# choi403/ALG

Measured on AMD Instinct MI355X. Metric: frames/sec (whole node) CogVideoX-5B-I2V 49f x 50-step ALG, higher is better.
Workload: dtype bf16; 1 GPU; BASELINE config 2: CogVideoX-5B-I2V bf16, 49 frames @ 480x720, 50 steps, ALG interval down_up (resize_factor 0.25, interval [0, 0.04]), guidance 6.0; one video per GPU; layers=42, dit_sample_forwards=12, parallelism=dp1

## Files before the change

alg_amd/_lib.py:

```python
from __future__ import annotations

import ctypes
from collections import OrderedDict
import os
from ctypes import POINTER, Structure, byref, c_char_p, c_float, c_int, c_int32, c_int64, c_void_p

import torch

_HERE = os.path.dirname(os.path.abspath(__file__))
LIB_PATH = os.environ.get("ALG_HIP_LIB") or os.path.join(_HERE, "libalg_hip.so")

ALG_F32, ALG_BF16 = 0, 1
ACT_NONE, ACT_GELU_TANH, ACT_SILU = 0, 1, 2
GEMM_BIAS_PER_ROW, GEMM_PERMUTE_COLS, GEMM_GATE_F32, GEMM_GATE_SEG_STRIDE = 1, 4, 8, 16
GEMM_B_PACKED11 = 32

EXPORTS = (
    "alg_version", "alg_last_error", "alg_reload_env", "alg_down_up", "alg_gaussian_blur", "alg_cfg_ddim_step", "alg_gemm_bf16", "alg_gemm_bf16_pair", "alg_gemm_bf16_pair_qk", "alg_pack_b_p11", "alg_pack_b_p11_bytes",
    "alg_flash_attn_d64", "alg_layernorm_modulate", "alg_layernorm_modulate_fp8", "alg_qk_norm_rope", "alg_patchify", "alg_unpatchify",
    "alg_timestep_embedding", "alg_cfg_combine", "alg_lincomb", "alg_unipc_update", "alg_concat_cast", "alg_flash_attn_d128", "alg_layernorm_mod_f32", "alg_layernorm_mod_f32_fp8", "alg_rmsnorm_rope",
    "alg_wan_modulation", "alg_patchify3d", "alg_unpatchify3d", "alg_timestep_embedding_f32", "alg_linear_f32",
    "alg_gelu_erf", "alg_layernorm_modulate_seg", "alg_headnorm_rope", "alg_masked_mean", "alg_silu", "alg_gemm_fp8", "alg_quantize_fp8_rows",
    "alg_conv_cl_bf16", "alg_vae_groupnorm_workspace", "alg_vae_groupnorm_stats", "alg_vae_spatial_norm", "alg_vae_upsample",
    "alg_vae_pack_latent", "alg_vae_unpack_video", "alg_vae_group_norm", "alg_vae_pad", "alg_vae_repitch",
    "alg_vae_unpack_planes", "alg_rms_norm_rows", "alg_softmax_hilo", "alg_flash_attn_d128_ex", "alg_flash_attn_d128_dual", "alg_rope_half", "alg_patchify_t", "alg_unpatchify_t", "alg_qk_norm_rope_scaled", "alg_flash_attn_d64_ex", "alg_embed_rows", "alg_t5_layernorm", "alg_attn_bias", "alg_mul_bf16", "alg_quick_gelu",
    "alg_lowpass_tables_bytes", "alg_lowpass_tables_build", "alg_down_up_workspace_bytes", "alg_gaussian_blur_workspace_bytes",
    "alg_flash_attn_d64_workspace_bytes", "alg_calib_mfma_bf16", "alg_wall_clock_khz", "alg_attn_clock_tap", "alg_attn_path_tap",
    "alg_flash_attn_d128_fp8", "alg_quantize_fp8_khead", "alg_quantize_fp8_vt", "alg_rmsnorm_rope_fp8", "alg_headnorm_rope_fp8",
    "alg_layernorm_modulate_seg_fp8", "alg_quantize_fp8_rows_batched", "alg_step_cache_probe", "alg_step_cache_workspace_bytes",
    "alg_flash_attn_d128_ranges", "alg_flash_attn_d64_ranges", "alg_flash_attn_d128_ranges_heads", "alg_attn_lse_recall", "alg_flash_attn_d64_ranges_heads",
    "alg_flash_attn_d128_ranges_order", "alg_flash_attn_d64_ranges_order",
    "alg_flash_attn_d128_ranges_prefix", "alg_attn_prefix_mass",
    "alg_gemm_fp4", "alg_quantize_mxfp4_rows", "alg_gemm_fp4_q4out", "alg_layernorm_modulate_mxfp4",
    "alg_attn_rows_position_major", "alg_attn_vt_position_major",
)
_RET_I64 = ("alg_vae_groupnorm_workspace", "alg_lowpass_tables_bytes", "alg_down_up_workspace_bytes",
            "alg_gaussian_blur_workspace_bytes", "alg_flash_attn_d64_workspace_bytes", "alg_pack_b_p11_bytes",
            "alg_step_cache_workspace_bytes")


class AlgHipError(RuntimeError):
    pass


class GemmArgs(Structure):
    _fields_ = [
        ("A", c_void_p), ("B", c_void_p), ("C", c_void_p), ("bias", c_void_p), ("R", c_void_p), ("gate", c_void_p),
        ("lda", c_int64), ("ldb", c_int64), ("ldc", c_int64), ("ldr", c_int64),
        ("strideA", c_int64), ("strideB", c_int64), ("strideC", c_int64), ("strideR", c_int64),
# ... 120 lines not shown
    lib.alg_t5_layernorm.argtypes = [c_void_p, c_void_p, c_void_p, c_int64, c_int, c_float, c_void_p]
    lib.alg_attn_bias.argtypes = [c_void_p] * 7 + [c_int, c_int, c_int, c_int, c_int64, c_int64, c_float, c_int, c_void_p]
    lib.alg_quick_gelu.argtypes = [c_void_p, c_int64, c_void_p]
    lib.alg_mul_bf16.argtypes = [c_void_p, c_void_p, c_void_p, c_int64, c_void_p]
    lib.alg_vae_upsample.argtypes = [c_void_p, c_void_p] + [c_int] * 6 + [c_void_p]
    lib.alg_vae_pack_latent.argtypes = [c_void_p, c_int64, c_int64, c_void_p, c_int, c_int, c_int, c_int, c_float, c_void_p]
    lib.alg_vae_unpack_video.argtypes = [c_void_p, c_void_p, c_int, c_int, c_int, c_int, c_void_p]
    lib.alg_quantize_fp8_rows.argtypes = [c_void_p, c_int64, c_void_p, c_void_p, c_int64, c_int, c_void_p]
    lib.alg_timestep_embedding_f32.argtypes = [c_void_p, c_void_p, c_int, c_int, c_void_p]
    lib.alg_linear_f32.argtypes = [c_void_p] * 6 + [c_int] * 4 + [c_void_p]
    lib.alg_gelu_erf.argtypes = [c_void_p, c_int64, c_void_p]
    lib.alg_unipc_update.argtypes = [c_void_p] * 5 + [c_int64] + [c_float] * 6 + [c_void_p]
    lib.alg_gemm_bf16.argtypes = [POINTER(GemmArgs), c_void_p]
    lib.alg_gemm_bf16_pair.argtypes = [POINTER(GemmArgs), POINTER(GemmArgs), c_void_p]
    lib.alg_gemm_bf16_pair_qk.argtypes = [POINTER(GemmArgs), POINTER(GemmArgs), POINTER(QkNormRopeArgs), c_void_p]
    lib.alg_flash_attn_d64.argtypes = [c_void_p, c_void_p, c_void_p, c_void_p, c_int, c_int, c_int, c_int64, c_int64,
                                       c_int64, c_int64, c_int64, c_int64, c_float, c_void_p]
    lib.alg_layernorm_modulate.argtypes = [c_void_p, c_void_p, c_void_p, c_void_p, c_void_p, c_void_p, c_int64, c_int,
                                           c_int, c_int, c_int64, c_int64, c_int, c_float, c_void_p]
    lib.alg_layernorm_modulate_fp8.argtypes = [c_void_p] * 7 + [c_int64, c_int, c_int, c_int, c_int64, c_int, c_float, c_void_p]
    lib.alg_layernorm_modulate_seg_fp8.argtypes = [c_void_p] * 7 + [c_int64, c_int64, c_int, c_int, c_int, c_int64, c_int, c_float,
                                                   c_void_p]
    lib.alg_quantize_fp8_rows_batched.argtypes = [c_void_p, c_int64, c_int64, c_void_p, c_void_p, c_int, c_int, c_int, c_void_p]
    lib.alg_qk_norm_rope.argtypes = [c_void_p, c_void_p, c_void_p, c_void_p, c_void_p, c_void_p, c_void_p, c_int,
                                     c_int, c_int, c_int, c_float, c_void_p]
    lib.alg_qk_norm_rope_scaled.argtypes = [c_void_p] * 7 + [c_int, c_int, c_int, c_int, c_float, c_float, c_void_p]
    lib.alg_flash_attn_d64_ex.argtypes = [c_void_p, c_void_p, c_void_p, c_void_p, c_int, c_int, c_int, c_int64, c_int64,
                                          c_int64, c_int64, c_int64, c_int64, c_float, c_int, c_void_p, c_int64, c_void_p]
    lib.alg_flash_attn_d64_ranges.argtypes = [c_void_p] * 4 + [c_int] * 3 + [c_int64] * 6 + [c_void_p, c_int, c_void_p]
    lib.alg_flash_attn_d64_ranges_heads.argtypes = ([c_void_p] * 4 + [c_int] * 3 + [c_int64] * 6 +
# ... 821 lines not shown
    lib = load_library()
    args, fp8 = gemm_args(*a, **kw)
    if fp8:
        _check(lib.alg_gemm_fp8(ctypes.byref(args), _stream()), "alg_gemm_fp8")
    else:
        _check(lib.alg_gemm_bf16(ctypes.byref(args), _stream()), "alg_gemm_bf16")


def gemm_pair(first, second):
    lib = load_library()
    a, fa = gemm_args(*first[0], **first[1])
    b, fb = gemm_args(*second[0], **second[1])
    if fa or fb:
        raise AlgHipError("gemm_pair takes bf16 problems")
    _check(lib.alg_gemm_bf16_pair(ctypes.byref(a), ctypes.byref(b), _stream()), "alg_gemm_bf16_pair")


def gemm_pair_qk(first, second, wq, bq, wk, bk, cos, sin, heads, text_len, eps, q_scale=1.0):
    lib = load_library()
    a, fa = gemm_args(*first[0], **first[1])
    b, fb = gemm_args(*second[0], **second[1])
    if fa or fb:
        raise AlgHipError("gemm_pair_qk takes bf16 problems")
    ptrs = [t.data_ptr() if t is not None else None for t in (wq, bq, wk, bk, cos, sin)]
    e = QkNormRopeArgs(*ptrs, heads, text_len, float(eps), float(q_scale))
    _check(lib.alg_gemm_bf16_pair_qk(ctypes.byref(a), ctypes.byref(b), ctypes.byref(e), _stream()), "alg_gemm_bf16_pair_qk")


def quantize_fp8_rows(x, q, scale, rows, K, x_rstride=None, x_off=0, q_off=0, scale_off=0):
    x_rstride = K if x_rstride is None else x_rstride
# ... 234 lines not shown
```

alg_amd/csrc/gemm.hip:

```cpp
#include <stdlib.h>

#include "common.h"

namespace alg {
constexpr int BM = 256, BN = 256;
typedef int launch_one_fn(const alg_gemm_args* a, int m_tiles, int n_tiles, int64_t nwg, hipStream_t s);
typedef int launch_pair_fn(const alg_gemm_args* a, int m_tiles_a, int n_tiles_a, const alg_gemm_args* b, int m_tiles_b, int n_tiles_b,
                           const alg_qk_norm_rope_args* e, hipStream_t s);
launch_one_fn launch_gemm_p6, launch_gemm_p6_conv, launch_gemm_p6_fp8, launch_gemm_p9, launch_gemm_p9_fp8, launch_gemm_p10, launch_gemm_p11;
launch_pair_fn launch_gemm_p9_pair, launch_gemm_p10_pair;
static int gemm_pipe() { return opt(OPT_GEMM_PIPE); }

static bool asm_loop_takes(int K, int64_t ld, int64_t esz) {
  return K * esz >= 256 && 256 * ld * esz + K * esz < (1ll << 32);
}

enum GemmRoute { ROUTE_P6, ROUTE_P6_CONV, ROUTE_P6_FP8, ROUTE_P9, ROUTE_P9_FP8, ROUTE_P10, ROUTE_P11 };
struct GemmPlan {
  GemmRoute route;
  int m_tiles, n_tiles;
  int64_t nwg;
  bool slabs;
  bool pairable;
};
}
// ... 160 lines not shown
}
static int pair_launch(const alg_gemm_args* a, const alg_gemm_args* b, const PairPlan& pp, const alg_qk_norm_rope_args* e, void* stream) {
  return (pp.a.route == ROUTE_P10 ? launch_gemm_p10_pair : launch_gemm_p9_pair)(a, pp.a.m_tiles, pp.a.n_tiles, b, pp.b.m_tiles,
                                                                                pp.b.n_tiles, e, (hipStream_t)stream);
}

extern "C" int alg_gemm_bf16_pair(const alg_gemm_args* a, const alg_gemm_args* b, void* stream) {
  PairPlan pp;
  int rc = pair_plan(a, b, &pp);
  if (rc != ALG_OK) return rc;
  if (pp.one_launch) return pair_launch(a, b, pp, nullptr, stream);
  rc = gemm_launch(a, pp.a, stream, false);
  return rc != ALG_OK ? rc : gemm_launch(b, pp.b, stream, false);
}

extern "C" int alg_gemm_bf16_pair_qk(const alg_gemm_args* a, const alg_gemm_args* b, const alg_qk_norm_rope_args* e, void* stream) {
  PairPlan pp;
  int rc = pair_plan(a, b, &pp);
  if (rc != ALG_OK) return rc;
  if (!e || !e->wq || !e->bq || !e->wk || !e->bk || e->heads <= 0 || e->text_len < 0 || e->text_len > a->M ||
      (e->cos_tab == nullptr) != (e->sin_tab == nullptr)) {
    set_error("alg_gemm_bf16_pair_qk: bad LayerNorm / rotary arguments");
    return ALG_EINVAL;
  }
  if (((uintptr_t)e->wq & 15) || ((uintptr_t)e->bq & 15) || ((uintptr_t)e->wk & 15) || ((uintptr_t)e->bk & 15) ||
      ((uintptr_t)e->cos_tab & 15) || ((uintptr_t)e->sin_tab & 15) || ((uintptr_t)a->C & 15)) {
    set_error("alg_gemm_bf16_pair_qk: pointers must be 16-byte aligned");
    return ALG_EINVAL;
  }
  if (a->N != 2 * e->heads * 64 || a->ldc != a->N || a->strideC != (int64_t)a->M * a->N || (a->flags & ALG_GEMM_PERMUTE_COLS) ||
// ... 41 lines not shown
```

alg_amd/csrc/gemm_kernel.h:

```cpp
#pragma once
#include <stdlib.h>

#include <type_traits>

#include "common.h"
#include "qk_norm_rope.h"
#ifdef ALG_P9_LOOP_INC
#include ALG_P9_LOOP_INC
#else
#include "gemm_p9_loop.inc"
#endif
#include "gemm_p9_fp8_loop.inc"
#ifdef ALG_P11_LOOP_INC
#include ALG_P11_LOOP_INC
#else
#include "gemm_p11_loop.inc"
#endif
#ifdef ALG_P10_LOOP_INC
#include ALG_P10_LOOP_INC
#else
#include "gemm_p10_loop.inc"
#endif

#ifndef ALG_FP8_MX
// ... 62 lines not shown
__device__ __forceinline__ void unpack4(const uint2 v, float (&f)[4]) {
  f[0] = __uint_as_float(v.x << 16);
  f[1] = __uint_as_float(v.x & 0xffff0000u);
  f[2] = __uint_as_float(v.y << 16);
  f[3] = __uint_as_float(v.y & 0xffff0000u);
}

struct GemmNoPair {};
struct GemmPairArgs {
  alg_gemm_args p;
  int m_tiles, n_tiles, group_m;
};
struct GemmPairQkArgs : GemmPairArgs {
  QkNormRope qe;
};
template <int PAIR> struct GemmPairT { typedef GemmNoPair type; };
template <> struct GemmPairT<1> { typedef GemmPairArgs type; };
template <> struct GemmPairT<2> { typedef GemmPairQkArgs type; };
template <int ACT, bool RES, int PIPE, int WNW = 4, bool FP8 = false, bool CONV = false, int PAIR = 0>
__global__ __launch_bounds__((PIPE == 11 ? 1 : 2) * WNW * 64) void gemm_bf16_kernel(
    const alg_gemm_args p1, int m_tiles1, int n_tiles1, int group_m1, const typename GemmPairT<PAIR>::type pr) {
  constexpr bool P9 = PIPE == 9 || PIPE == 10 || PIPE == 11;
  constexpr bool M16 = PIPE == 10 || PIPE == 11;
  constexpr bool P11 = PIPE == 11;
  constexpr int WMW = P11 ? 1 : 2;
  constexpr int MT = BM / WMW / 32;
  static_assert(!PAIR || (P9 && !P11 && !RES && ACT == ALG_ACT_NONE), "the pair launch is built for the plain schedule-9 / 10 kernels");
  static_assert(!FP8 || PIPE == 6 || PIPE == 9, "the fp8 operands are built on the ping-pong schedule and on schedule 9");
  static_assert(!CONV || (PIPE == 6 && !FP8), "the convolution addressing is built on the bf16 ping-pong schedule");
  typedef typename std::conditional<FP8, uint8_t, bf16_t>::type elem_t;
  constexpr int EPS = 16 / (int)sizeof(elem_t);
  constexpr int GEMM_THREADS = WMW * WNW * 64;
  constexpr int NT = BN / WNW / 32;
  static_assert(PIPE == 6 || P9, "schedules built: 6 (ping-pong), 9 / 10 / 11 (asm loops)");
  static_assert((PIPE == 9 || PIPE == 10) == (WNW == 2) && P11 == (WNW == 4 && WMW == 1),
                "PIPE 9 / 10 are the 2 x 2 4-wave layouts, 11 the 1 x 4 one, 6 runs 8 waves");
  static_assert(!P11 || (!FP8 && !CONV), "schedule 11 takes bf16 plain GEMM addressing with a packed B");
  static_assert(!P9 || !CONV, "schedules 9 / 10 take plain GEMM addressing (bf16, or e4m3 on 9 since round 4)");
  constexpr bool PP = PIPE == 6;
  constexpr int BK = FP8 ? 128 : 64;
  constexpr int ROW_BYTES = BK * (int)sizeof(elem_t);
  constexpr int SLOTS = ROW_BYTES / 16;
// ... 5 lines not shown

  extern __shared__ __attribute__((aligned(16))) char smem[];
  const int tid = threadIdx.x;
  const int lane = tid & 63;
  const int wave = __builtin_amdgcn_readfirstlane(tid >> 6);
  const int wm = wave / WNW, wn = wave % WNW;

#ifdef ALG_GEMM_TAP
  uint64_t tap_loop = 0, tap_tiles = 0;
  const uint64_t tap_c0 = __builtin_readcyclecounter(), tap_r0 = wall_clock64();
#endif
  group_m1 &= 0xffff;
  const int total1 = m_tiles1 * n_tiles1 * p1.batch;
  auto do_tile = [&](const int wg_in) __attribute__((always_inline)) {
  bool second = false;
  if constexpr (PAIR) second = wg_in >= total1;
  const alg_gemm_args& p = [&]() -> const alg_gemm_args& {
    if constexpr (PAIR) return second ? pr.p : p1;
    else return p1;
  }();
  int m_tiles = m_tiles1, n_tiles = n_tiles1, group_m = group_m1, wg = wg_in;
  if constexpr (PAIR) {
    if (second) m_tiles = pr.m_tiles, n_tiles = pr.n_tiles, group_m = pr.group_m, wg = wg_in - total1;
  }
  const int tiles = m_tiles * n_tiles;
  const int b = wg / tiles;
  int t = wg - b * tiles;
  const int grp = t / (group_m * n_tiles);
  const int first_m = grp * group_m;
  const int gsize = min(m_tiles - first_m, group_m);
  t -= grp * group_m * n_tiles;
  const int m0 = (first_m + t % gsize) * BM;
  const int n0 = (t / gsize) * BN;

  const elem_t* A = (const elem_t*)p.A + (int64_t)b * p.strideA;
  const elem_t* B = (const elem_t*)p.B + (int64_t)b * p.strideB;

// ... 311 lines not shown
      ALG_P9_STATEMENT(ALG_GEMM_P9_FP8_LOOP_ASM, ALG_GEMM_P9_CLOBBERS);
    } else if constexpr (M16) {
      ALG_P9_STATEMENT(ALG_GEMM_P10_LOOP_ASM, ALG_GEMM_P10_CLOBBERS);
    } else {
      ALG_P9_STATEMENT(ALG_GEMM_P9_LOOP_ASM, ALG_GEMM_P9_CLOBBERS);
    }
#undef ALG_P9_STATEMENT
#endif
    }
#ifdef ALG_GEMM_TAP
    tap_loop += __builtin_readcyclecounter() - tap_l0s, ++tap_tiles;
#endif
    __builtin_amdgcn_s_barrier();
  }

  const bf16_t* bias = (const bf16_t*)p.bias;
  const bf16_t* R = RES ? (const bf16_t*)p.R + (int64_t)b * p.strideR : nullptr;
  const bf16_t* gate = (RES && p.gate) ? (const bf16_t*)p.gate + (int64_t)b * p.strideGate : nullptr;
  const bool bias_row = p.flags & ALG_GEMM_BIAS_PER_ROW;
  const bool perm = p.flags & ALG_GEMM_PERMUTE_COLS;
  const int64_t gate_seg = (p.flags & ALG_GEMM_GATE_SEG_STRIDE) ? p.gate_seg_stride : p.N;
  const bool gate_f32 = RES && p.gate && (p.flags & ALG_GEMM_GATE_F32);
  bf16_t* Cb = (bf16_t*)p.C + (int64_t)b * p.strideC;
  const int ldc = (int)p.ldc, ldr = (int)p.ldr;
  const int col0 = perm ? p.perm_col0 : 0;
  const bool n_vec = (p.N & 3) == 0 && (col0 & 15) == 0;
  auto blk_row = [&](int mt) { return PP ? (mt >> 1) * 128 + wm * 64 + (mt & 1) * 32 : wm * (MT * 32) + mt * 32; };
  auto blk_col = [&](int nt) { return PP ? nt * 128 + wn * 32 : wn * (NT * 32) + nt * 32; };
  auto quad_row = [](int q, int ln_) { return M16 ? 16 * (q >> 1) + (ln_ & 15) : (ln_ & 31); };
  auto quad_col = [](int q, int ln_) { return M16 ? 16 * (q & 1) + 4 * (ln_ >> 4) : 8 * q + 4 * (ln_ >> 5); };
// ... 505 lines not shown
              const int nj = nn + col0;
              const int nc = perm ? ((nj & ~12) | ((nj & 4) << 1) | ((nj & 8) >> 1)) : nn;
              Cb[row * ldc + nc] = f2bf(x);
            }
          }
        }
      }
    });
  };
#ifndef ALG_EPI_STAGED_ONLY
  static_for<MT>([&](auto mt_c) { epilogue_band(mt_c); });
#endif
  };

  int total_wg = total1;
  if constexpr (PAIR) total_wg += pr.m_tiles * pr.n_tiles * pr.p.batch;
  for (int L = blockIdx.x; L < total_wg; L += gridDim.x) {
    const int xcd = L & 7, q = total_wg >> 3, r = total_wg & 7;
    const int wg = (xcd < r ? xcd * (q + 1) : r * (q + 1) + (xcd - r) * q) + (L >> 3);
    if (L != (int)blockIdx.x) __syncthreads();
    do_tile(wg);
  }
#ifdef ALG_GEMM_TAP
  if (threadIdx.x == 0 && blockIdx.x < 1024) {
    uint64_t* t = gemm_tap_buf + blockIdx.x * 4;
    t[0] = __builtin_readcyclecounter() - tap_c0, t[1] = wall_clock64() - tap_r0, t[2] = tap_loop, t[3] = tap_tiles;
  }
#endif
}

inline unsigned gemm_grid(int64_t nwg) {
// ... 31 lines not shown
    hipLaunchKernelGGL((gemm_bf16_kernel<ALG_ACT_NONE, true, PIPE, WNW, FP8>), grid, block, LDS, s, *a, m_tiles,
                       n_tiles, gm, GemmNoPair{});
  } else if (a->act == ALG_ACT_GELU_TANH) {
    hipLaunchKernelGGL((gemm_bf16_kernel<ALG_ACT_GELU_TANH, false, PIPE, WNW, FP8>), grid, block, LDS, s, *a, m_tiles,
                       n_tiles, gm, GemmNoPair{});
  } else if (a->act == ALG_ACT_SILU) {
    hipLaunchKernelGGL((gemm_bf16_kernel<ALG_ACT_SILU, false, PIPE, WNW, FP8>), grid, block, LDS, s, *a, m_tiles,
                       n_tiles, gm, GemmNoPair{});
  } else {
    hipLaunchKernelGGL((gemm_bf16_kernel<ALG_ACT_NONE, false, PIPE, WNW, FP8>), grid, block, LDS, s, *a, m_tiles,
                       n_tiles, gm, GemmNoPair{});
  }
  return check_launch("alg_gemm_bf16");
}

template <int PIPE, int PAIR>
int launch_gemm_pair(const alg_gemm_args* a, int m_tiles_a, int n_tiles_a, const alg_gemm_args* b, int m_tiles_b, int n_tiles_b,
                     const alg_qk_norm_rope_args* e, hipStream_t s) {
  static_assert(PAIR == 1 || PAIR == 2, "a pair, or a pair whose first problem is the Q|K projection");
  const auto kernel = gemm_bf16_kernel<ALG_ACT_NONE, false, PIPE, 2, false, false, PAIR>;
  const char* const entry = PAIR == 2 ? "alg_gemm_bf16_pair_qk" : "alg_gemm_bf16_pair";
  static PerDeviceOnce attr_set;
  const int rc = opt_in_lds(attr_set, {(const void*)kernel}, GEMM_LDS_P9, entry);
  if (rc != ALG_OK) return rc;
  const int64_t nwg = (int64_t)m_tiles_a * n_tiles_a * a->batch + (int64_t)m_tiles_b * n_tiles_b * b->batch;
  typename GemmPairT<PAIR>::type pr;
  pr.p = *b, pr.m_tiles = m_tiles_b, pr.n_tiles = n_tiles_b, pr.group_m = gemm_group_m(PIPE, n_tiles_b, b->K) & 0xffff;
  if constexpr (PAIR == 2) {
    pr.qe.wq = (const bf16_t*)e->wq, pr.qe.bq = (const bf16_t*)e->bq, pr.qe.wk = (const bf16_t*)e->wk, pr.qe.bk = (const bf16_t*)e->bk;
    pr.qe.cos_tab = e->cos_tab, pr.qe.sin_tab = e->sin_tab, pr.qe.heads = e->heads, pr.qe.text_len = e->text_len;
// ... 8 lines not shown
```

alg_amd/csrc/gemm_p11.hip:

```cpp
#include "gemm_kernel.h"

namespace alg {
int launch_gemm_p11(const alg_gemm_args* a, int m_tiles, int n_tiles, int64_t nwg, hipStream_t s) {
  return launch_gemm<11, 4>(a, m_tiles, n_tiles, nwg, s);
}

__global__ __launch_bounds__(256) void pack_b_p11_kernel(const bf16_t* __restrict__ w, uint4* __restrict__ out, int N, int K, int64_t ldb,
                                                          int64_t total) {
  const int64_t i = (int64_t)blockIdx.x * 256 + threadIdx.x;
  if (i >= total) return;
  const int lane = (int)(i & 63);
  const int f = (int)((i >> 6) & 7), wv = (int)((i >> 9) & 3);
  const int64_t tile = i >> 11;
  const int nkt = K / 64;
  const int kt = (int)(tile % nkt);
  const int64_t nt = tile / nkt;
  const int n = (int)(nt * 256) + wv * 64 + (f & 3) * 16 + (lane & 15);
  const int k = kt * 64 + (f >> 2) * 32 + (lane >> 4) * 8;
  uint4 v = make_uint4(0u, 0u, 0u, 0u);
  if (n < N) v = *(const uint4*)(w + (int64_t)n * ldb + k);
  out[i] = v;
}
}

// ... 22 lines not shown
```

alg_amd/transformer_cogvideox.py:

```python
from __future__ import annotations

import math
import os
from dataclasses import dataclass, asdict
from typing import Optional

import torch

from . import _lib
from .attn_window import HeadWindowHost, SelfAttnOperands, calibrate_self_attention, launch_self_attention
from .step_cache import StepCacheHost


@dataclass
class CogVideoXTransformerConfig:

    num_attention_heads: int = 48
    attention_head_dim: int = 64
    in_channels: int = 32
    out_channels: int = 16
    num_layers: int = 42
    time_embed_dim: int = 512
    text_embed_dim: int = 4096
    max_text_seq_length: int = 226
# ... 14 lines not shown
    spatial_interpolation_scale: float = 1.875
    temporal_interpolation_scale: float = 1.0

    @property
    def inner_dim(self):
        return self.num_attention_heads * self.attention_head_dim

    def to_dict(self):
        return asdict(self)


def _bf(t, device):
    return t.to(device=device, dtype=torch.bfloat16).contiguous()


class CogVideoXTransformer3DModel(StepCacheHost, HeadWindowHost):
    dtype = torch.bfloat16

    FP8_WEIGHTS = ("wqk", "wv", "wo", "wf1", "wf2")

    FP4_WEIGHTS = ("wf1", "wf2")

    def __init__(self, config: CogVideoXTransformerConfig, weights: dict, device="cuda", fp8=False, fp4=False):
        cfg = self.config = config
        self.device = torch.device(device)
        if self.device.type != "cuda":
            raise _lib.AlgHipError("CogVideoXTransformer3DModel runs on the GPU only (HIP kernels, no CPU fallback)")
        if cfg.attention_head_dim != 64:
            raise _lib.AlgHipError("the attention kernel is specialised for head_dim 64")
        if cfg.ofs_embed_dim is not None and cfg.ofs_embed_dim != cfg.time_embed_dim:
# ... 1 lines not shown
        D = cfg.inner_dim
        if D % 512:
            raise _lib.AlgHipError("inner_dim must be a multiple of 512 (LayerNorm kernel tiling)")
        self.fp8 = bool(fp8)
        if self.fp8:
            self._check_fp8_shapes()
        self.fp4 = bool(fp4)
        if self.fp4:
            self._check_fp4_shapes()
        self.fuse_quant = True
        _lib.load_library()
        self.attn_prescale = True
        self.pair_qkv = True
        self.fuse_qk_norm = False
        self.packed_weights = True
        self.step_cache = 0.0
        self.step_cache_max_consecutive = 0
        self.attn_window = 0
        self.attn_sink_frames = 1
        self._head_window_init()
        self._sincos = {}
        dev = self.device
        w = weights
        p = cfg.patch_size
        self.p_t = cfg.patch_size_t or 1
        self.k_patch = cfg.in_channels * p * p * self.p_t
        if self.k_patch % 64 or cfg.text_embed_dim % 64 or cfg.time_embed_dim % 64:
            raise _lib.AlgHipError("GEMM K dimensions must be multiples of 64")
        self.w_patch = _bf(w["patch_embed.proj.weight"].reshape(D, self.k_patch), dev)
        self.b_patch = _bf(w["patch_embed.proj.bias"], dev)
# ... 31 lines not shown
                L[nm + "_b"] = _bf(w[b + "attn1." + nm + ".bias"], dev)
            L["wo"] = _bf(w[b + "attn1.to_out.0.weight"], dev)
            L["bo"] = _bf(w[b + "attn1.to_out.0.bias"], dev)
            L["wf1"] = _bf(w[b + "ff.net.0.proj.weight"], dev)
            L["bf1"] = _bf(w[b + "ff.net.0.proj.bias"], dev)
            L["wf2"] = _bf(w[b + "ff.net.2.weight"], dev)
            L["bf2"] = _bf(w[b + "ff.net.2.bias"], dev)
            if self.fp4:
                self._quantize_layer_fp4(L, drop_bf16=True)
            if self.fp8:
                self._quantize_layer(L, drop_bf16=True)
            else:
                for nm in ("wo", "wf1", "wf2"):
                    if nm in L:
                        L["p" + nm] = _lib.PackedB(L[nm])
            self.layers.append(L)
        ow, ob = w["norm_out.linear.weight"], w["norm_out.linear.bias"]
        sh_w, sc_w = ow.chunk(2, dim=0)
        sh_b, sc_b = ob.chunk(2, dim=0)
        mw.append(torch.cat([sh_w, sh_w, sc_w, sc_w], dim=0))
        mb.append(torch.cat([sh_b, sh_b, sc_b, sc_b], dim=0))
        self.w_mod = _bf(torch.cat(mw, dim=0), dev)
        self.b_mod = _bf(torch.cat(mb, dim=0), dev)
        self.mod_cols = self.w_mod.shape[0]
        self.norm_final_w = _bf(w["norm_final.weight"], dev)
        self.norm_final_b = _bf(w["norm_final.bias"], dev)
        self.norm_out_w = _bf(w["norm_out.norm.weight"], dev)
        self.norm_out_b = _bf(w["norm_out.norm.bias"], dev)
        self.w_out = _bf(w["proj_out.weight"], dev)
        self.b_out = _bf(w["proj_out.bias"], dev)
# ... 81 lines not shown
        from .weights import synthetic_state_dict

        config = config or CogVideoXTransformerConfig()
        return cls(config, synthetic_state_dict(config, seed=seed, std=std, device=device,
                                                 randomize_affine=randomize_affine), device=device, fp8=fp8, fp4=fp4)

    @classmethod
    def from_pretrained(cls, path, subfolder="transformer", torch_dtype=torch.bfloat16, device="cuda", fp8=False, fp4=False, **_):
        from .weights import load_diffusers_transformer

        config, sd = load_diffusers_transformer(path, subfolder)
        return cls(config, sd, device=device, fp8=fp8, fp4=fp4)

    def to(self, *args, **kwargs):
        return self

    def _workspace(self, N, S, P):
        key = (N, S, P)
        ws = self._ws.get(key)
        if ws is not None:
            return ws
        cfg, dev = self.config, self.device
        D = cfg.inner_dim
        bf = dict(device=dev, dtype=torch.bfloat16)
        S_pad = (S + 127) // 128 * 128
        ws = dict(
            S_pad=S_pad,
            x=torch.empty(N, S, D, **bf),
            y=torch.empty(N, S, D, **bf),
            qk=torch.empty(N, S, 2 * D, **bf),
# ... 219 lines not shown
            _lib.silu(emb, ws["semb"])
        G(ws["semb"], self.w_mod, mod, N, self.mod_cols, E, E, E, self.mod_cols, bias=self.b_mod)

        G(ehs, self.w_text, x, T, D, cfg.text_embed_dim, cfg.text_embed_dim, cfg.text_embed_dim, D,
          bias=self.b_text, R=pos_emb, ldr=D, batch=N, strideA=T * cfg.text_embed_dim, strideC=S * D)
        _lib.patchify(lat, 0 if Bl == 1 else Fr * C * Hh * Ww, conds, ws["patches"], N, Fr, C, Hh, Ww, p, p_t)
        G(ws["patches"], self.w_patch, x, P, D, self.k_patch, self.k_patch, self.k_patch, D, bias=self.b_patch,
          R=pos_emb, ldr=D, r_off=T * D, batch=N, strideA=P * self.k_patch, strideC=S * D, c_off=T * D)

        scale = 1.0 / math.sqrt(cfg.attention_head_dim)
        prescale = self.attn_prescale
        q_scale = scale * 1.4426950408889634 if prescale else 1.0
        F4 = cfg.ff_inner_mult * D
        packed = self.packed_weights and os.environ.get("ALG_GEMM_PIPE", "10") == "10"
        wo_k, wf1_k, wf2_k = ("pwo", "pwf1", "pwf2") if packed else ("wo", "wf1", "wf2")
        kvr = self._window_ranges(Fr // p_t, (Hh // p) * (Ww // p), T) if self.attn_window else None
        sc = self._step_cache_begin(x, cache_keys, cache_force, T, P)
        plan = self._self_attn_begin([kvr], (Fr // p_t, (Hh // p) * (Ww // p), T, int(self.attn_window), int(self.attn_sink_frames)),
                                     len(self.layers), N, Hn, S, (N, S, D), batch=N)
        for li, L in enumerate(self.layers):
            if li == 1 and sc is not None and TM("step_cache", sc.after_block0, x):
                break
            m1 = li * 12 * D
            m2 = m1 + 6 * D
            if fp8:
                self._block_fp8(L, ws, q8, q8s, N, S, T, m1, m2, cos, sin, scale, q_scale, prescale, plan, li, fp4)
                continue
            TM("ln_mod", _lib.layernorm_modulate, x, y, L["norm1_w"], L["norm1_b"], mod, mod, self.mod_cols, N, S, D,
               T, cfg.norm_eps, scale_off=m1 + 2 * D, shift_off=m1)
            qk_call = ((y, L["wqk"], qk, S, 2 * D, D, D, D, 2 * D), dict(bias=L["bqk"], batch=N, strideA=S * D, strideC=S * 2 * D))
            vt_call = ((L["wv"], y, vt, D, S, D, D, D, S_pad), dict(bias=L["bv"], batch=N, strideB=S * D, strideC=D * S_pad,
                                                                   flags=_lib.GEMM_BIAS_PER_ROW | _lib.GEMM_PERMUTE_COLS))
            if self.pair_qkv and self.fuse_qk_norm:
                TM("gemm_qkv", _lib.gemm_pair_qk, qk_call, vt_call, L["norm_q_w"], L["norm_q_b"], L["norm_k_w"], L["norm_k_b"], cos, sin,
                               Hn, T, cfg.qk_norm_eps, q_scale=q_scale)
            else:
                if self.pair_qkv:
                    TM("gemm_qkv", _lib.gemm_pair, qk_call, vt_call)
                else:
                    TM("gemm_qk", G, *qk_call[0], **qk_call[1])
                    TM("gemm_vt", G, *vt_call[0], **vt_call[1])
                TM("qk_norm_rope", _lib.qk_norm_rope_, qk, L["norm_q_w"], L["norm_q_b"], L["norm_k_w"], L["norm_k_b"], cos, sin, N, S, Hn, T,
                                   cfg.qk_norm_eps, q_scale=q_scale)
            self._attention(ws, plan, li, N, S, T, scale, prescale)
            TM("gemm_out", G, att, L[wo_k], x, S, D, D, D, D, D, bias=L["bo"], R=x, ldr=D, gate=mod, gate_off=m1 + 4 * D,
              strideGate=self.mod_cols, seg_split=T, batch=N, strideA=S * D, strideC=S * D, strideR=S * D)
            if fp4:
                self._ff_fp4(L, ws, N, S, T, m2)
# ... 44 lines not shown
```

include/alg_hip.h:

```cpp
#ifndef ALG_HIP_H
#define ALG_HIP_H

#include <stdint.h>

#ifdef __cplusplus
extern "C" {
#endif

#define ALG_F32 0
#define ALG_BF16 1

#define ALG_OK 0
#define ALG_EINVAL (-1)
#define ALG_ELAUNCH (-2)
#define ALG_ELIMIT (-3)

#define ALG_VERSION 110

int alg_version(void);
const char* alg_last_error(void);

void alg_reload_env(void);


// ... 61 lines not shown
  const float* b_scale;
  int64_t strideAScale, strideBScale;
  int32_t conv_wp;
  int32_t conv_hpwp;
  int32_t conv_kw;
  int32_t reserved1;
} alg_gemm_args;

int alg_gemm_bf16(const alg_gemm_args* args, void* stream);

int64_t alg_pack_b_p11_bytes(int N, int K);
int alg_pack_b_p11(const void* w, void* packed, int N, int K, int64_t ldb, void* stream);

int alg_gemm_bf16_pair(const alg_gemm_args* a, const alg_gemm_args* b, void* stream);

typedef struct alg_qk_norm_rope_args {
  const void *wq, *bq, *wk, *bk;
  const float *cos_tab, *sin_tab;
  int32_t heads, text_len;
  float eps, q_scale;
} alg_qk_norm_rope_args;
int alg_gemm_bf16_pair_qk(const alg_gemm_args* qk, const alg_gemm_args* vt, const alg_qk_norm_rope_args* e, void* stream);

int alg_gemm_fp8(const alg_gemm_args* args, void* stream);

int alg_quantize_fp8_rows(const void* x, int64_t x_rstride, void* q, float* scale, int64_t rows, int K, void* stream);
int alg_gemm_fp4(const alg_gemm_args* args, void* stream);

int alg_quantize_mxfp4_rows(const void* x, int64_t x_rstride, void* q, void* scales, int64_t rows, int K, void* stream);

// ... 240 lines not shown
```

Measured before the change: 1.477 frames/s.

## Fuse QKV projection into one packed GEMM with transposed V column-split epilogue

Replaces the paired QK and V^T GEMMs with one schedule-11 GEMM over a concatenated, pre-packed QKV weight. Column tiles past the split point stage their accumulators through LDS and write V transposed into the attention V^T buffer. Column tiles before it use the normal epilogue into the QK buffer. The goal is to read the normalized activations once, use the faster packed-B schedule, and drop a launch. In exchange it stores an extra packed copy of the QKV weights per layer and adds a new, complex transposed epilogue with alignment constraints.

```diff
diff --git a/alg_amd/_lib.py b/alg_amd/_lib.py
--- a/alg_amd/_lib.py
+++ b/alg_amd/_lib.py
@@ -33,6 +33,7 @@
     "alg_flash_attn_d128_ranges_prefix", "alg_attn_prefix_mass",
     "alg_gemm_fp4", "alg_quantize_mxfp4_rows", "alg_gemm_fp4_q4out", "alg_layernorm_modulate_mxfp4",
     "alg_attn_rows_position_major", "alg_attn_vt_position_major",
+    "alg_gemm_bf16_split",
 )
 _RET_I64 = ("alg_vae_groupnorm_workspace", "alg_lowpass_tables_bytes", "alg_down_up_workspace_bytes",
             "alg_gaussian_blur_workspace_bytes", "alg_flash_attn_d64_workspace_bytes", "alg_pack_b_p11_bytes",
@@ -183,6 +184,7 @@
     lib.alg_gemm_bf16.argtypes = [POINTER(GemmArgs), c_void_p]
     lib.alg_gemm_bf16_pair.argtypes = [POINTER(GemmArgs), POINTER(GemmArgs), c_void_p]
     lib.alg_gemm_bf16_pair_qk.argtypes = [POINTER(GemmArgs), POINTER(GemmArgs), POINTER(QkNormRopeArgs), c_void_p]
+    lib.alg_gemm_bf16_split.argtypes = [POINTER(GemmArgs), c_void_p, c_int64, c_int64, c_int32, c_void_p]
     lib.alg_flash_attn_d64.argtypes = [c_void_p, c_void_p, c_void_p, c_void_p, c_int, c_int, c_int, c_int64, c_int64,
                                        c_int64, c_int64, c_int64, c_int64, c_float, c_void_p]
     lib.alg_layernorm_modulate.argtypes = [c_void_p, c_void_p, c_void_p, c_void_p, c_void_p, c_void_p, c_int64, c_int,
@@ -1034,6 +1036,14 @@
     if fa or fb:
         raise AlgHipError("gemm_pair takes bf16 problems")
     _check(lib.alg_gemm_bf16_pair(ctypes.byref(a), ctypes.byref(b), _stream()), "alg_gemm_bf16_pair")
+
+
+def gemm_split(first, Ct, ldct, strideCt, n_split, ct_off=0):
+    lib = load_library()
+    a, fa = gemm_args(*first[0], **first[1])
+    if fa:
+        raise AlgHipError("gemm_split takes a bf16 problem")
+    _check(lib.alg_gemm_bf16_split(ctypes.byref(a), Ct.data_ptr() + 2 * ct_off, ldct, strideCt, n_split, _stream()), "alg_gemm_bf16_split")
 
 
 def gemm_pair_qk(first, second, wq, bq, wk, bk, cos, sin, heads, text_len, eps, q_scale=1.0):
diff --git a/alg_amd/csrc/gemm.hip b/alg_amd/csrc/gemm.hip
--- a/alg_amd/csrc/gemm.hip
+++ b/alg_amd/csrc/gemm.hip
@@ -9,6 +9,8 @@
                            const alg_qk_norm_rope_args* e, hipStream_t s);
 launch_one_fn launch_gemm_p6, launch_gemm_p6_conv, launch_gemm_p6_fp8, launch_gemm_p9, launch_gemm_p9_fp8, launch_gemm_p10, launch_gemm_p11;
 launch_pair_fn launch_gemm_p9_pair, launch_gemm_p10_pair;
+int launch_gemm_p11_split(const alg_gemm_args* a, void* Ct, int64_t ldct, int64_t strideCt, int n_split, int m_tiles, int n_tiles,
+                          int64_t nwg, hipStream_t s);
 static int gemm_pipe() { return opt(OPT_GEMM_PIPE); }
 
 static bool asm_loop_takes(int K, int64_t ld, int64_t esz) {
@@ -199,6 +201,64 @@
   return rc != ALG_OK ? rc : gemm_launch(b, pp.b, stream, false);
 }
 
+static bool ranges_overlap(const void* p, int64_t pbytes, const void* q, int64_t qbytes) {
+  const uintptr_t a = (uintptr_t)p, b = (uintptr_t)q;
+  return a < b + (uintptr_t)qbytes && b < a + (uintptr_t)pbytes;
+}
+static int split_check(const alg_gemm_args* a, const void* Ct, int64_t ldct, int64_t strideCt, int n_split) {
+  const int rc = gemm_check(a, false);
+  if (rc != ALG_OK) return rc;
+  if (!(a->flags & ALG_GEMM_B_PACKED11)) {
+    set_error("alg_gemm_bf16_split: B must be packed for schedule 11 (alg_pack_b_p11, ALG_GEMM_B_PACKED11)");
+    return ALG_EINVAL;
+  }
+  if (a->a_scale || a->b_scale) {
+    set_error("alg_gemm_bf16_split: bf16 operands only (a_scale / b_scale belong to the e4m3 GEMM)");
+    return ALG_EINVAL;
+  }
+  if (a->R || a->gate || a->act != ALG_ACT_NONE) {
+    set_error("alg_gemm_bf16_split: the column split is a plain GEMM (no residual, gate or activation)");
+    return ALG_EINVAL;
+  }
+  if (n_split <= 0 || n_split % BN || n_split >= a->N || a->N % 8 || n_split > a->ldc) {
+    set_error("alg_gemm_bf16_split: n_split=%d must be a positive multiple of %d below N=%d (N %% 8 == 0) and fit a row of C (ldc=%lld)",
+              n_split, BN, a->N, (long long)a->ldc);
+    return ALG_EINVAL;
+  }
+  const int64_t m64 = ((int64_t)a->M + 63) / 64 * 64;
+  if (!Ct || ((uintptr_t)Ct & 15) || ldct < m64 || ldct % 8 || strideCt % 8 || strideCt < 0 || ((uintptr_t)a->C & 15) || a->ldc % 8 ||
+      a->strideC % 8) {
+    set_error("alg_gemm_bf16_split: Ct / C must be 16-byte aligned with ldct=%lld >= M rounded up to 64 (%lld) and ldct / ldc / batch "
+              "strides multiples of 8 elements", (long long)ldct, (long long)m64);
+    return ALG_EINVAL;
+  }
+  if (a->batch > 1 && strideCt < (int64_t)(a->N - n_split) * ldct) {
+    set_error("alg_gemm_bf16_split: the batch items of Ct overlap (strideCt=%lld < %d rows of %lld)", (long long)strideCt, a->N - n_split,
+              (long long)ldct);
+    return ALG_EINVAL;
+  }
+  const int64_t nb = a->batch - 1;
+  const int64_t ct_bytes = (nb * strideCt + (int64_t)(a->N - n_split) * ldct) * 2;
+  const int64_t a_bytes = (nb * a->strideA + (int64_t)(a->M - 1) * a->lda + a->K) * 2;
+  const int64_t c_bytes = (nb * a->strideC + (int64_t)(a->M - 1) * a->ldc + n_split) * 2;
+  if (ranges_overlap(Ct, ct_bytes, a->A, a_bytes) || ranges_overlap(Ct, ct_bytes, a->C, c_bytes)) {
+    set_error("alg_gemm_bf16_split: Ct overlaps A or C");
+    return ALG_EINVAL;
+  }
+  return ALG_OK;
+}
+
+extern "C" int alg_gemm_bf16_split(const alg_gemm_args* a, void* Ct, int64_t ldct, int64_t strideCt, int32_t n_split, void* stream) {
+  const int rc = split_check(a, Ct, ldct, strideCt, n_split);
+  if (rc != ALG_OK) return rc;
+  const GemmPlan p = gemm_plan(a, false);
+  if (p.slabs || p.nwg > 0x7fffffff) {
+    set_error("alg_gemm_bf16_split: M*ldc must stay below 2^31 (32-bit epilogue offsets of the C tiles; the split is not cut into slabs)");
+    return ALG_ELIMIT;
+  }
+  return launch_gemm_p11_split(a, Ct, ldct, strideCt, n_split, p.m_tiles, p.n_tiles, p.nwg, (hipStream_t)stream);
+}
+
 extern "C" int alg_gemm_bf16_pair_qk(const alg_gemm_args* a, const alg_gemm_args* b, const alg_qk_norm_rope_args* e, void* stream) {
   PairPlan pp;
   int rc = pair_plan(a, b, &pp);
diff --git a/alg_amd/csrc/gemm_kernel.h b/alg_amd/csrc/gemm_kernel.h
--- a/alg_amd/csrc/gemm_kernel.h
+++ b/alg_amd/csrc/gemm_kernel.h
@@ -100,9 +100,16 @@
 struct GemmPairQkArgs : GemmPairArgs {
   QkNormRope qe;
 };
+struct GemmSplitArgs {
+  void* Ct;
+  int64_t ldct, strideCt;
+  int n_split;
+};
 template <int PAIR> struct GemmPairT { typedef GemmNoPair type; };
 template <> struct GemmPairT<1> { typedef GemmPairArgs type; };
 template <> struct GemmPairT<2> { typedef GemmPairQkArgs type; };
+template <> struct GemmPairT<3> { typedef GemmSplitArgs type; };
+constexpr int SPLIT_PITCH = 528, SPLIT_WAVE_BYTES = 64 * SPLIT_PITCH;
 template <int ACT, bool RES, int PIPE, int WNW = 4, bool FP8 = false, bool CONV = false, int PAIR = 0>
 __global__ __launch_bounds__((PIPE == 11 ? 1 : 2) * WNW * 64) void gemm_bf16_kernel(
     const alg_gemm_args p1, int m_tiles1, int n_tiles1, int group_m1, const typename GemmPairT<PAIR>::type pr) {
@@ -111,7 +118,11 @@
   constexpr bool P11 = PIPE == 11;
   constexpr int WMW = P11 ? 1 : 2;
   constexpr int MT = BM / WMW / 32;
-  static_assert(!PAIR || (P9 && !P11 && !RES && ACT == ALG_ACT_NONE), "the pair launch is built for the plain schedule-9 / 10 kernels");
+  constexpr bool TWO = PAIR == 1 || PAIR == 2;
+  constexpr bool SPLIT = PAIR == 3;
+  static_assert(!TWO || (P9 && !P11 && !RES && ACT == ALG_ACT_NONE), "the pair launch is built for the plain schedule-9 / 10 kernels");
+  static_assert(!SPLIT || (P11 && !RES && ACT == ALG_ACT_NONE), "the column split is built for the plain schedule-11 kernel");
+  static_assert(PAIR >= 0 && PAIR <= 3, "PAIR: 0 | 1 | 2 (two problems) | 3 (column split)");
   static_assert(!FP8 || PIPE == 6 || PIPE == 9, "the fp8 operands are built on the ping-pong schedule and on schedule 9");
   static_assert(!CONV || (PIPE == 6 && !FP8), "the convolution addressing is built on the bf16 ping-pong schedule");
   typedef typename std::conditional<FP8, uint8_t, bf16_t>::type elem_t;
@@ -147,13 +158,13 @@
   const int total1 = m_tiles1 * n_tiles1 * p1.batch;
   auto do_tile = [&](const int wg_in) __attribute__((always_inline)) {
   bool second = false;
-  if constexpr (PAIR) second = wg_in >= total1;
+  if constexpr (TWO) second = wg_in >= total1;
   const alg_gemm_args& p = [&]() -> const alg_gemm_args& {
-    if constexpr (PAIR) return second ? pr.p : p1;
+    if constexpr (TWO) return second ? pr.p : p1;
     else return p1;
   }();
   int m_tiles = m_tiles1, n_tiles = n_tiles1, group_m = group_m1, wg = wg_in;
-  if constexpr (PAIR) {
+  if constexpr (TWO) {
     if (second) m_tiles = pr.m_tiles, n_tiles = pr.n_tiles, group_m = pr.group_m, wg = wg_in - total1;
   }
   const int tiles = m_tiles * n_tiles;
@@ -495,6 +506,69 @@
     __builtin_amdgcn_s_barrier();
   }
 
+  if constexpr (SPLIT) {
+    if (n0 >= pr.n_split) {
+      int z = 0;
+      asm volatile("" : "+s"(z));
+      const int le = __builtin_amdgcn_mbcnt_hi(~0u, __builtin_amdgcn_mbcnt_lo(~0u, z));
+      char* const my = smem + wave * SPLIT_WAVE_BYTES;
+      const int l15 = le & 15;
+      const int pl = (l15 & 3) | ((l15 & 4) << 1) | ((l15 & 8) >> 1);
+      char* const park = my + 4 * (le >> 4) * SPLIT_PITCH + pl * 2;
+      static_for<MT>([&](auto mt_c) {
+        constexpr int mt = decltype(mt_c)::value;
+        static_for<NT>([&](auto nt_c) {
+          constexpr int nt = decltype(nt_c)::value;
+          const f32x16 blk = get_acc(mt_c, nt_c);
+#pragma unroll
+          for (int g = 0; g < 4; ++g) {
+            float bv[4];
+            unpack4(bcol_early[nt][g & 1], bv);
+            const uint32_t p01 = pack_bf2(blk[4 * g] + bv[0], blk[4 * g + 1] + bv[1]);
+            const uint32_t p23 = pack_bf2(blk[4 * g + 2] + bv[2], blk[4 * g + 3] + bv[3]);
+            char* const q = park + (nt * 32 + 16 * (g & 1)) * SPLIT_PITCH + (mt * 32 + 16 * (g >> 1)) * 2;
+            *(bf16_t*)q = (bf16_t)p01;
+            *(bf16_t*)(q + SPLIT_PITCH) = (bf16_t)(p01 >> 16);
+            *(bf16_t*)(q + 2 * SPLIT_PITCH) = (bf16_t)p23;
+            *(bf16_t*)(q + 3 * SPLIT_PITCH) = (bf16_t)(p23 >> 16);
+          }
+        });
+      });
+      asm volatile("s_waitcnt lgkmcnt(0)" ::: "memory");
+      bf16_t* const Ctb = (bf16_t*)pr.Ct + (int64_t)b * pr.strideCt;
+      const int ch = le & 31, fr0 = le >> 5;
+      const int j = m0 + ch * 8;
+      const int t0 = (j & ~12) | ((j & 8) >> 1);
+      const bool full = t0 + 11 < p.M, some = t0 < p.M;
+      static_for<4>([&](auto grp_c) {
+        constexpr int g0 = decltype(grp_c)::value * 8;
+        uint4 raw[8];
+        static_for<8>([&](auto j_c) {
+          constexpr int it = g0 + decltype(j_c)::value;
+          raw[decltype(j_c)::value] = *(const uint4*)(my + (it * 2 + fr0) * SPLIT_PITCH + ch * 16);
+        });
+        static_for<8>([&](auto j_c) {
+          constexpr int it = g0 + decltype(j_c)::value;
+          const int n = n0 + wn * 64 + it * 2 + fr0;
+          const uint4 v = raw[decltype(j_c)::value];
+          bf16_t* const dst = Ctb + (int64_t)(n - pr.n_split) * pr.ldct + j;
+          if (n < p.N) {
+            if (full) {
+              ALG_STORE16(dst, v);
+            } else if (some) {
+              const uint32_t u[4] = {v.x, v.y, v.z, v.w};
+#pragma unroll
+              for (int e = 0; e < 8; ++e)
+                if (t0 + (e & 3) + ((e >> 2) << 3) < p.M) dst[e] = (bf16_t)(u[e >> 1] >> ((e & 1) * 16));
+            }
+          }
+        });
+        __builtin_amdgcn_sched_barrier(0);
+      });
+      return;
+    }
+  }
+
   const bf16_t* bias = (const bf16_t*)p.bias;
   const bf16_t* R = RES ? (const bf16_t*)p.R + (int64_t)b * p.strideR : nullptr;
   const bf16_t* gate = (RES && p.gate) ? (const bf16_t*)p.gate + (int64_t)b * p.strideGate : nullptr;
@@ -1030,7 +1104,7 @@
   };
 
   int total_wg = total1;
-  if constexpr (PAIR) total_wg += pr.m_tiles * pr.n_tiles * pr.p.batch;
+  if constexpr (TWO) total_wg += pr.m_tiles * pr.n_tiles * pr.p.batch;
   for (int L = blockIdx.x; L < total_wg; L += gridDim.x) {
     const int xcd = L & 7, q = total_wg >> 3, r = total_wg & 7;
     const int wg = (xcd < r ? xcd * (q + 1) : r * (q + 1) + (xcd - r) * q) + (L >> 3);
@@ -1092,6 +1166,20 @@
   return check_launch("alg_gemm_bf16");
 }
 
+template <int PIPE>
+int launch_gemm_split(const alg_gemm_args* a, void* Ct, int64_t ldct, int64_t strideCt, int n_split, int m_tiles, int n_tiles,
+                             int64_t nwg, hipStream_t s) {
+  static_assert(4 * SPLIT_WAVE_BYTES <= GEMM_LDS_P9, "four transposed wave tiles fit the ring");
+  const auto kernel = gemm_bf16_kernel<ALG_ACT_NONE, false, PIPE, 4, false, false, 3>;
+  static PerDeviceOnce attr_set;
+  const int rc = opt_in_lds(attr_set, {(const void*)kernel}, GEMM_LDS_P9, "alg_gemm_bf16_split");
+  if (rc != ALG_OK) return rc;
+  GemmSplitArgs sp;
+  sp.Ct = Ct, sp.ldct = ldct, sp.strideCt = strideCt, sp.n_split = n_split;
+  hipLaunchKernelGGL(kernel, dim3(gemm_grid(nwg)), dim3(256), GEMM_LDS_P9, s, *a, m_tiles, n_tiles, gemm_group_m(PIPE, n_tiles, a->K), sp);
+  return check_launch("alg_gemm_bf16_split");
+}
+
 template <int PIPE, int PAIR>
 int launch_gemm_pair(const alg_gemm_args* a, int m_tiles_a, int n_tiles_a, const alg_gemm_args* b, int m_tiles_b, int n_tiles_b,
                      const alg_qk_norm_rope_args* e, hipStream_t s) {
diff --git a/alg_amd/csrc/gemm_p11.hip b/alg_amd/csrc/gemm_p11.hip
--- a/alg_amd/csrc/gemm_p11.hip
+++ b/alg_amd/csrc/gemm_p11.hip
@@ -3,6 +3,10 @@
 namespace alg {
 int launch_gemm_p11(const alg_gemm_args* a, int m_tiles, int n_tiles, int64_t nwg, hipStream_t s) {
   return launch_gemm<11, 4>(a, m_tiles, n_tiles, nwg, s);
+}
+int launch_gemm_p11_split(const alg_gemm_args* a, void* Ct, int64_t ldct, int64_t strideCt, int n_split, int m_tiles, int n_tiles,
+                          int64_t nwg, hipStream_t s) {
+  return launch_gemm_split<11>(a, Ct, ldct, strideCt, n_split, m_tiles, n_tiles, nwg, s);
 }
 
 __global__ __launch_bounds__(256) void pack_b_p11_kernel(const bf16_t* __restrict__ w, uint4* __restrict__ out, int N, int K, int64_t ldb,
diff --git a/alg_amd/transformer_cogvideox.py b/alg_amd/transformer_cogvideox.py
--- a/alg_amd/transformer_cogvideox.py
+++ b/alg_amd/transformer_cogvideox.py
@@ -52,6 +52,9 @@
     return t.to(device=device, dtype=torch.bfloat16).contiguous()
 
 
+SPLIT_QKV_DEFAULT = True
+
+
 class CogVideoXTransformer3DModel(StepCacheHost, HeadWindowHost):
     dtype = torch.bfloat16
 
@@ -83,6 +86,7 @@
         self.pair_qkv = True
         self.fuse_qk_norm = False
         self.packed_weights = True
+        self.split_qkv = SPLIT_QKV_DEFAULT
         self.step_cache = 0.0
         self.step_cache_max_consecutive = 0
         self.attn_window = 0
@@ -144,6 +148,8 @@
                 for nm in ("wo", "wf1", "wf2"):
                     if nm in L:
                         L["p" + nm] = _lib.PackedB(L[nm])
+                if self.split_qkv and D % 128 == 0:
+                    self._pack_qkv(L)
             self.layers.append(L)
         ow, ob = w["norm_out.linear.weight"], w["norm_out.linear.bias"]
         sh_w, sc_w = ow.chunk(2, dim=0)
@@ -255,6 +261,13 @@
 
     def to(self, *args, **kwargs):
         return self
+
+    @staticmethod
+    def _pack_qkv(L):
+        if "pwqkv" not in L:
+            L["pwqkv"] = _lib.PackedB(torch.cat([L["wqk"], L["wv"]], dim=0))
+            L["bqkv"] = torch.cat([L["bqk"], L["bv"]], dim=0)
+        return L["pwqkv"]
 
     def _workspace(self, N, S, P):
         key = (N, S, P)
@@ -504,6 +517,7 @@
         F4 = cfg.ff_inner_mult * D
         packed = self.packed_weights and os.environ.get("ALG_GEMM_PIPE", "10") == "10"
         wo_k, wf1_k, wf2_k = ("pwo", "pwf1", "pwf2") if packed else ("wo", "wf1", "wf2")
+        split_qkv = packed and self.split_qkv and self.pair_qkv and not self.fuse_qk_norm and D % 128 == 0
         kvr = self._window_ranges(Fr // p_t, (Hh // p) * (Ww // p), T) if self.attn_window else None
         sc = self._step_cache_begin(x, cache_keys, cache_force, T, P)
         plan = self._self_attn_begin([kvr], (Fr // p_t, (Hh // p) * (Ww // p), T, int(self.attn_window), int(self.attn_sink_frames)),
@@ -521,7 +535,12 @@
             qk_call = ((y, L["wqk"], qk, S, 2 * D, D, D, D, 2 * D), dict(bias=L["bqk"], batch=N, strideA=S * D, strideC=S * 2 * D))
             vt_call = ((L["wv"], y, vt, D, S, D, D, D, S_pad), dict(bias=L["bv"], batch=N, strideB=S * D, strideC=D * S_pad,
                                                                    flags=_lib.GEMM_BIAS_PER_ROW | _lib.GEMM_PERMUTE_COLS))
-            if self.pair_qkv and self.fuse_qk_norm:
+            if split_qkv:
+                TM("gemm_qkv", _lib.gemm_split, ((y, self._pack_qkv(L), qk, S, 3 * D, D, D, D, 2 * D),
+                                                 dict(bias=L["bqkv"], batch=N, strideA=S * D, strideC=S * 2 * D)), vt, S_pad, D * S_pad, 2 * D)
+                TM("qk_norm_rope", _lib.qk_norm_rope_, qk, L["norm_q_w"], L["norm_q_b"], L["norm_k_w"], L["norm_k_b"], cos, sin, N, S, Hn, T,
+                                   cfg.qk_norm_eps, q_scale=q_scale)
+            elif self.pair_qkv and self.fuse_qk_norm:
                 TM("gemm_qkv", _lib.gemm_pair_qk, qk_call, vt_call, L["norm_q_w"], L["norm_q_b"], L["norm_k_w"], L["norm_k_b"], cos, sin,
                                Hn, T, cfg.qk_norm_eps, q_scale=q_scale)
             else:
diff --git a/include/alg_hip.h b/include/alg_hip.h
--- a/include/alg_hip.h
+++ b/include/alg_hip.h
@@ -99,6 +99,8 @@
 
 int alg_gemm_bf16_pair(const alg_gemm_args* a, const alg_gemm_args* b, void* stream);
 
+int alg_gemm_bf16_split(const alg_gemm_args* args, void* Ct, int64_t ldct, int64_t strideCt, int32_t n_split, void* stream);
+
 typedef struct alg_qk_norm_rope_args {
   const void *wq, *bq, *wk, *bk;
   const float *cos_tab, *sin_tab;
```

Result: no change. 1.486 frames/s, median of 6 (+0.6%).
